# stecrotti/MatrixProductBP.jl

Hardware: AMD Instinct MI355X
Metric: edge-message updates/sec (and s/sweep), SIS 3-regular N=1024 T=50 d=20 (higher is better)
Workload: dtype f64

## Files before the change

### matrixproductbp.jl_amd/csrc/engine.h

```cpp
#if !defined(WG_THREADS)
#error "engine.h is included from kernels.h, once per workgroup-size variant"
#endif

namespace eng {

using namespace wg;

__device__ __forceinline__ int r16(int x) { return (x + 15) & ~15; }
__device__ __forceinline__ int r32(int x) { return (x + 31) & ~31; }

typedef __attribute__((address_space(1))) int32_t gint;
typedef __attribute__((address_space(3))) int lint;

template <class DP>
__device__ inline void stage_core(DP dst, const gdbl* base, const gint* bond, int64_t stride, int L,
                                  int t, bool mirror, int nyq) {
  const int tp = mirror ? (L - 1 - t) : t;
  const int pl = bond[tp], pr = bond[tp + 1];
  const int a = mirror ? pr : pl, an = mirror ? pl : pr;
  const gdbl* src = base + (int64_t)tp * stride;
  const int tot = a * an * nyq;
  for (int idx = threadIdx.x; idx < tot; idx += WG_THREADS) {
    int m = idx % a; int rest = idx / a; int n = rest % an; int s = rest / an;
    int mp = mirror ? n : m, np_ = mirror ? m : n;
    dst[idx] = src[mp + pl * (np_ + pr * s)];
  }
}

template <class DP>
__device__ inline void build_E(DP E, DP A2c, const gdbl* pyy, int b, int bn, int ny, int ny1,
                               int ny2, int q) {
  const int M2 = b * ny, K2 = bn * ny1;
  const int tot = M2 * K2 * q;
  for (int idx = threadIdx.x; idx < tot; idx += WG_THREADS) {
    int i = idx % M2; int rest = idx / M2; int kk = rest % K2; int xi = rest / K2;
    int m2 = i % b, y = i / b, n2 = kk % bn, y1 = kk / bn;
    double s = 0.0;
    for (int y2 = 0; y2 < ny2; y2++) {
      double c = pyy[y + ny * (y1 + ny1 * (y2 + ny2 * xi))];
      if (c != 0.0) s += c * A2c[m2 + b * (n2 + bn * (y2 + ny2 * xi))];
    }
    E[idx] = s;
  }
}

__device__ inline void atomic_max_double_pos(unsigned long long* addr, double v) {
  atomicMax(addr, (unsigned long long)__double_as_longlong(v));
}

template <bool CORES_LDS, bool JAC_LDS, bool EXT>
__device__ void run_problem(const EngProb& P, const EngCfg& cfg, double* slot_, double* lds_, EngStats* stats) {
  typedef typename std::conditional<CORES_LDS, ldbl*, gdbl*>::type CP;
  typedef typename std::conditional<JAC_LDS, ldbl*, gdbl*>::type JP;
  const int tid = threadIdx.x;
  const int L = cfg.L;
  const bool mirror = P.mirror != 0;
  const int ny1 = P.ny1, ny2 = P.ny2, ny = P.ny, q = P.q;
  gdbl* slot = (gdbl*)slot_;
  ldbl* lds = (ldbl*)lds_;
  ldbl* ldsG = lds + cfg.lds_gemm;
  ldbl* ldsQ = lds + cfg.lds_qr;
  ldbl* misc = lds + cfg.lds_misc;
  CP A1c = CORES_LDS ? (CP)(lds + cfg.lds_A1c) : (CP)(slot + cfg.off_A1c);
  CP A2c = CORES_LDS ? (CP)(lds + cfg.lds_A2c) : (CP)(slot + cfg.off_A2c);
  CP E = CORES_LDS ? (CP)(lds + cfg.lds_E) : (CP)(slot + cfg.off_E);
  JP JA = JAC_LDS ? (JP)(lds + cfg.lds_JA) : (JP)(slot + cfg.off_JA);
  lint* rdim = (lint*)(lds + cfg.lds_rdim);
  ldbl* red = misc;
  ldbl* sig = misc + 32;
  lint* ord = (lint*)(misc + 32 + cfg.nmax);
  gdbl* LfS = slot + cfg.off_Lf;
  gdbl* Z = slot + cfg.off_Z;
  gdbl* Y = slot + cfg.off_Y;
  gdbl* T1 = slot + cfg.off_T1;
  gdbl* Nt = slot + cfg.off_Nt;
  gdbl* Mt = slot + cfg.off_Mt;
  gdbl* Ccur = slot + cfg.off_C0;
  gdbl* Cnew = slot + cfg.off_C1;
  const gdbl* PA1 = (const gdbl*)P.A1; const gdbl* PA2 = (const gdbl*)P.A2;
  const gint* Pb1 = (const gint*)P.bond1; const gint* Pb2 = (const gint*)P.bond2;
  const gdbl* Ppyy = (const gdbl*)P.pyy;
  gdbl* Pout = (gdbl*)P.out; gint* Pob = (gint*)P.obond;

  auto LB1 = [&](int t) { return mirror ? Pb1[L - t] : Pb1[t]; };
  auto LB2 = [&](int t) { return mirror ? Pb2[L - t] : Pb2[t]; };
  auto TP = [&](int t) { return mirror ? (L - 1 - t) : t; };
  constexpr bool ext = EXT;
  const gdbl* Plf = (const gdbl*)P.lf;
  const __attribute__((address_space(1))) int64_t* Plfoff = (const __attribute__((address_space(1))) int64_t*)P.lfoff;
  const gint* Prd = (const gint*)P.rdim;
  auto RD = [&](int t) -> int { return ext ? (int)Prd[t] : (int)rdim[t]; };
  auto LFP = [&](int t) -> const gdbl* { return ext ? Plf + Plfoff[t] : (const gdbl*)(LfS + (int64_t)t * cfg.lf_stride); };
  Prof* pr = cfg.prof;
  unsigned long long plast = pr ? wall_clock64() : 0ULL;
#define PROF(ph) prof_mark(pr, plast, ph)

  if (tid == 0 && !ext) { rdim[L] = 1; LfS[(int64_t)L * cfg.lf_stride] = 1.0; }
  __syncthreads();
  for (int t = ext ? 0 : L - 1; t >= 1; t--) {
    const int a = LB1(t), an = LB1(t + 1), b = LB2(t), bn = LB2(t + 1);
    const int Bm = a * b, Bn = an * bn;
    const int r1 = rdim[t + 1];
    const gdbl* Lf1 = LfS + (int64_t)(t + 1) * cfg.lf_stride;
    stage_core(A1c, PA1, Pb1, P.stride1, L, t, mirror, ny1 * q);
    stage_core(A2c, PA2, Pb2, P.stride2, L, t, mirror, ny2 * q);
    __syncthreads();
    build_E(E, A2c, Ppyy + (int64_t)TP(t) * P.pyy_tstride, b, bn, ny, ny1, ny2, q);
    __syncthreads();
    PROF(PH_STAGE);
    const int M1 = a * ny1 * q;
    const int64_t zld = (int64_t)r1 * bn;
    gemm_direct<false, true>(M1, r1 * bn, an, A1c,
         [=](int i) { return (i % a) + a * an * (i / a); }, [=](int kk) { return a * kk; },
         Lf1, [=](int kk) { return (int64_t)r1 * kk; },
         [=](int j) { return (int64_t)(j % r1) + (int64_t)r1 * an * (j / r1); },
         Z, [=](int i) { return zld * i; }, [=](int j) { return (int64_t)j; }, false);
    PROF(PH_Y1);
    const int rowsY = r1 * ny * q;
    const int ldY = r32(rowsY);
    const int cols16 = r16(Bm) + 16;
    for (int64_t idx = tid; idx < (int64_t)(ldY - rowsY) * cols16; idx += WG_THREADS) {
      int rr = rowsY + (int)(idx % (ldY - rowsY)); int64_t c = idx / (ldY - rowsY);
      Y[rr + (int64_t)ldY * c] = 0.0;
    }
    for (int64_t idx = tid; idx < (int64_t)ldY * (cols16 - Bm); idx += WG_THREADS)
      Y[(int64_t)ldY * Bm + idx] = 0.0;
    const int M2 = b * ny, K2 = bn * ny1;
    for (int xi = 0; xi < q; xi++) {
      gemm_direct<true, true>(M2, r1 * a, K2, E + (int64_t)xi * M2 * K2,
           [=](int i) { return i; }, [=](int kk) { return M2 * kk; },
           Z + zld * a * ny1 * xi,
           [=](int kk) { return (int64_t)r1 * (kk % bn) + zld * a * (kk / bn); },
           [=](int j) { return (int64_t)(j % r1) + zld * (j / r1); },
           Y + (int64_t)r1 * ny * xi,
           [=](int i) { return (int64_t)r1 * (i / b) + (int64_t)ldY * a * (i % b); },
           [=](int j) { return (int64_t)(j % r1) + (int64_t)ldY * (j / r1); }, false);
    }
    PROF(PH_Y2);
    qr_r(Y, ldY, rowsY, Bm, ldsQ, ldsG, pr, &plast, PH_QR1_PANEL, PH_QR1_TRAIL, cfg.force_generic != 0);
    const int kmax = min(rowsY, Bm);
    const int lane_ = tid & 63, wave_ = __builtin_amdgcn_readfirstlane(tid >> 6);
    constexpr int LFC = 4;
    double mx = 0.0;
    for (int m0 = LFC * wave_; m0 < Bm; m0 += LFC * WG_WAVES) {
      const int kcap = min(kmax, m0 + LFC);
      for (int k = lane_; k < kcap; k += 64) {
        double v[LFC];
#pragma unroll
        for (int c = 0; c < LFC; c++) {
          const int m = min(m0 + c, Bm - 1);
          v[c] = Y[(int64_t)ldY * m + min(k, min(kmax, m + 1) - 1)];
        }
#pragma unroll
        for (int c = 0; c < LFC; c++) mx = fmax(mx, fabs(v[c]));
      }
    }
    mx = wg_max(mx, red);
    const double inv = (mx > 0.0 && isfinite(mx)) ? 1.0 / mx : 1.0;
    gdbl* Lf0 = LfS + (int64_t)t * cfg.lf_stride;
    for (int m0 = LFC * wave_; m0 < Bm; m0 += LFC * WG_WAVES) {
      for (int k = lane_; k < kmax; k += 64) {
        double v[LFC];
#pragma unroll
        for (int c = 0; c < LFC; c++) {
          const int m = min(m0 + c, Bm - 1);
          v[c] = Y[(int64_t)ldY * m + min(k, min(kmax, m + 1) - 1)];
        }
#pragma unroll
        for (int c = 0; c < LFC; c++) {
          const int m = m0 + c;
          if (m < Bm) Lf0[(int64_t)kmax * m + k] = (k < min(kmax, m + 1)) ? v[c] * inv : 0.0;
        }
      }
    }
    if (tid == 0) rdim[t] = kmax;
    __syncthreads();
    PROF(PH_LF);
  }

  double logc = 0.0;
  int kc = 1;
  if (tid == 0) Ccur[0] = 1.0;
  if (tid == 0) { Pob[mirror ? L : 0] = 1; Pob[mirror ? 0 : L] = 1; }
  __syncthreads();
  for (int t = 0; t < L; t++) {
    const int a = LB1(t), an = LB1(t + 1), b = LB2(t), bn = LB2(t + 1);
    const int Bn = an * bn;
    const int tp = TP(t);
    stage_core(A1c, PA1, Pb1, P.stride1, L, t, mirror, ny1 * q);
// ... 3 lines not shown
    __syncthreads();
    PROF(PH_STAGE);
    const int MT1 = an * ny1 * q;
    const int64_t tld = (int64_t)kc * b;
    gemm_direct(MT1, kc * b, a, A1c,
         [=](int i) { return a * (i % an) + a * an * (i / an); }, [=](int kk) { return kk; },
         Ccur, [=](int kk) { return (int64_t)kc * kk; },
         [=](int j) { return (int64_t)(j % kc) + (int64_t)kc * a * (j / kc); },
         T1, [=](int i) { return tld * i; }, [=](int j) { return (int64_t)j; }, false);
    const int Rr = kc * ny * q;
    const int M2 = b * ny, K2 = bn * ny1;
    for (int xi = 0; xi < q; xi++) {
      gemm_direct(bn * ny, kc * an, b * ny1, E + (int64_t)xi * M2 * K2,
           [=](int i) { return b * (i / bn) + M2 * (i % bn); },
           [=](int kk) { return (kk % b) + M2 * bn * (kk / b); },
           T1 + tld * an * ny1 * xi,
           [=](int kk) { return (int64_t)kc * (kk % b) + tld * an * (kk / b); },
           [=](int j) { return (int64_t)(j % kc) + tld * (j / kc); },
           Nt + (int64_t)kc * ny * xi,
           [=](int i) { return (int64_t)kc * (i / bn) + (int64_t)Rr * an * (i % bn); },
           [=](int j) { return (int64_t)(j % kc) + (int64_t)Rr * (j / kc); }, false);
    }
    {
      double mx = wg_maxabs(Nt, Rr, Rr, Bn, red);
      if (!(mx == mx) || isinf(mx)) { if (tid == 0) stats->nan_flag = 1; }
      if (mx > 0.0 && isfinite(mx)) {
        const double inv = 1.0 / mx;
        for (int64_t idx = tid; idx < (int64_t)Rr * Bn; idx += WG_THREADS) Nt[idx] *= inv;
        logc += log(mx);
      }
      __syncthreads();
    }
    PROF(PH_N);
    gdbl* oc = Pout + (int64_t)tp * P.ostride;
    if (t == L - 1) {
      for (int idx = tid; idx < Rr; idx += WG_THREADS) {
        int k = idx % kc, s = idx / kc;
        oc[k + kc * s] = Nt[idx];
      }
      __syncthreads();
      break;
    }
    const int r1 = RD(t + 1);
    const gdbl* Lf1 = LFP(t + 1);
    const int ldM = r32(r1);
    const int Rr16 = r16(Rr) + 16;
    for (int64_t idx = tid; idx < (int64_t)(ldM - r1) * Rr16; idx += WG_THREADS) {
      int rr = r1 + (int)(idx % (ldM - r1)); int64_t c = idx / (ldM - r1);
      Mt[rr + (int64_t)ldM * c] = 0.0;
    }
    for (int64_t idx = tid; idx < (int64_t)ldM * (Rr16 - Rr); idx += WG_THREADS) Mt[(int64_t)ldM * Rr + idx] = 0.0;
    gemm(Rr, r1, Bn, Nt, [=](int i) { return (int64_t)i; }, [=](int kk) { return (int64_t)Rr * kk; },
         Lf1, [=](int kk) { return (int64_t)r1 * kk; }, [=](int j) { return j; }, false,
         Mt, [=](int i) { return (int64_t)ldM * i; }, [=](int j) { return j; }, false, ldsG);
    PROF(PH_MT);
    qr_r(Mt, ldM, r1, Rr, ldsQ, ldsG, pr, &plast, PH_QR2_PANEL, PH_QR2_TRAIL, cfg.force_generic != 0);
    const int k2 = min(r1, Rr);
    const int ldJ = JAC_LDS ? (Rr | 1) : ((Rr + 15) & ~15);
    double fro2 = 0.0;
    for (int idx = tid; idx < k2 * Rr; idx += WG_THREADS) {
      int r = idx % Rr, c = idx / Rr;
      double v = (r >= c) ? Mt[c + (int64_t)ldM * r] : 0.0;
      JA[r + ldJ * c] = v;
      fro2 += v * v;
    }
    fro2 = wg_sum(fro2, red);
    __syncthreads();
    const int sw = jacobi_rsv(JA, ldJ, Rr, k2, nullptr, 0, red, ord, 60);
    if (tid == 0) {
      if (sw < 0) stats->jacobi_fail = 1;
      atomicAdd(&stats->jac_sweeps, (unsigned long long)(sw < 0 ? 60 : sw));
      atomicAdd(&stats->jac_calls, 1ULL);
    }
    PROF(PH_JAC);
    const double nul2 = 1e-28 * fro2;
    for (int c = tid; c < Rr; c += WG_THREADS) sig[c] = 0.0;
    __syncthreads();
    for (int c = tid; c < k2; c += WG_THREADS) {
      double s = 0.0;
      for (int r = 0; r < Rr; r++) { double v = JA[r + ldJ * c]; s += v * v; }
      const bool ok = s > nul2 && s > 0.0;
      const double sg = ok ? sqrt(s) : 0.0, inv = ok ? 1.0 / sqrt(s) : 0.0;
      for (int r = 0; r < Rr; r++) JA[r + ldJ * c] *= inv;
      sig[c] = sg;
    }
    __syncthreads();
    for (int c = tid; c < k2; c += WG_THREADS) {
      const double sc = sig[c];
      int rank = 0;
      for (int j = 0; j < k2; j++) { double sj = sig[j]; rank += (sj > sc) || (sj == sc && j < c); }
      ord[rank] = c;
    }
    __syncthreads();
    const int len = min(Rr, r1);
    int kp;
    {
      double tot = 0.0;
      for (int j = 0; j < len; j++) { double s = sig[ord[j]]; tot += s * s; }
      const mpbp_trunc tr = cfg.trunc;
      int kth = len;
      if (tr.kind == MPBP_TRUNC_THRESH || tr.kind == MPBP_TRUNC_BOND_THRESH) {
        const double thr = tr.eps * sqrt(tot);
        kth = 0;
        for (int j = 0; j < len; j++) if (sig[ord[j]] > thr) kth = j + 1;
        if (kth < 1) kth = 1;
      }
      if (tr.kind == MPBP_TRUNC_THRESH) kp = kth;
// ... 54 lines not shown
```

### matrixproductbp.jl_amd/csrc/mpbp_hip.hip

```cpp
#include <chrono>
#include "kernels.h"
#include "ctx.h"
#include "v2_engine.h"

thread_local std::string g_create_error;

extern "C" const char* mpbp_last_error(const mpbp_ctx* ctx) { return ctx ? ctx->err.c_str() : g_create_error.c_str(); }

extern "C" int mpbp_create(mpbp_ctx** out, const mpbp_desc* d) {
  if (!out || !d) { g_create_error = "null argument"; return MPBP_EINVAL; }
  *out = nullptr;
  if (d->n_nodes <= 0 || d->n_edges <= 0 || d->T < 1 || d->q < 1 || d->q > 4 || d->max_bond < 1 || !d->nbr_ptr ||
      !d->in_edge || !d->out_edge) { g_create_error = "invalid descriptor (need n_nodes,n_edges>0, T>=1, 1<=q<=4, max_bond>=1)"; return MPBP_EINVAL; }
  mpbp_ctx* c = new mpbp_ctx();
  c->N = d->n_nodes; c->E = d->n_edges; c->T = d->T; c->L = d->T + 1; c->q = d->q; c->cap = d->max_bond; c->device = d->device; c->periodic = d->periodic != 0;
  c->nbr_ptr.assign(d->nbr_ptr, d->nbr_ptr + c->N + 1);
  const int nnz = c->nbr_ptr[c->N];
  c->in_edge.assign(d->in_edge, d->in_edge + nnz);
  c->out_edge.assign(d->out_edge, d->out_edge + nnz);
  for (int p = 0; p < nnz; p++)
    if (c->in_edge[p] < 0 || c->in_edge[p] >= c->E || c->out_edge[p] < 0 || c->out_edge[p] >= c->E) {
      g_create_error = "edge id out of range"; delete c; return MPBP_EINVAL;
    }
  c->nslots = d->n_slots > 0 ? d->n_slots : c->E;
// ... 352 lines not shown
      std::vector<double> w((size_t)L * q * q * q * nyc);
      for (int t = 0; t < L; t++)
        for (int y1 = 0; y1 < nyc; y1++)
          for (int xj = 0; xj < q; xj++)
            for (int x = 0; x < q; x++)
              for (int xn = 0; xn < q; xn++) {
                double val;
                if (xj >= QD(eo)) val = 0.0;
                else if (t == L - 1 && !c->periodic) val = PHI(i, t, x);
                else {
                  double s = 0.0;
                  for (int y = 0; y < nyz; y++)
                    for (int y2 = 0; y2 < ny1; y2++) {
                      const double pyy = PYY(t, z - 1, 1, y, y1, y2, x);
                      if (pyy != 0.0) s += PY(t, xn, x, y) * PXY(t, k, y2, xj, x) * pyy;
                    }
                  val = s * PHI(i, t, x);
                }
                w[(size_t)t * q * q * q * nyc + xn + q * (x + q * (xj + (size_t)q * y1))] = val;
              }
      c->wmsg_off[p] = ts.add(w);
    }
    {
      std::vector<double> w((size_t)L * q * q * nyz);
      for (int t = 0; t < L; t++)
        for (int y = 0; y < nyz; y++)
          for (int x = 0; x < q; x++)
            for (int xn = 0; xn < q; xn++)
              w[(size_t)t * q * q * nyz + xn + q * (x + (size_t)q * y)] = (t == L - 1 && !c->periodic) ? PHI(i, t, x) : PY(t, xn, x, y) * PHI(i, t, x);
      c->wbel_off[i] = ts.add(w);
    }
  }
  if (c->d_tab) { hipFree(c->d_tab); c->d_tab = nullptr; }
  c->tab_doubles = ts.data.size();
  HIPCHK(c, hipMalloc(&c->d_tab, sizeof(double) * std::max<size_t>(ts.data.size(), 4)));
  HIPCHK(c, hipMemcpy(c->d_tab, ts.data.data(), sizeof(double) * ts.data.size(), hipMemcpyHostToDevice));
  c->tables_dirty = false;
  return MPBP_OK;
}

#define RCCHK(call) do { const int rc_ = (call); if (rc_ != MPBP_OK) return rc_; } while (0)

namespace {

enum Form { FORM_AUTO, FORM_GRID, FORM_WG };

struct SweepEnv {
  int split_nodes = 0;
  bool force_generic = false;
  bool no_small = false;
  bool force_small = false;
  bool no_pack = false;
  bool coop_fail_once = false;
  Form gauge = FORM_AUTO, sweep2 = FORM_AUTO;
};
static SweepEnv read_sweep_env() {
  auto set = [](const char* name) { return getenv(name) != nullptr; };
  auto is1 = [](const char* name) { const char* e = getenv(name); return e && e[0] == '1'; };
  auto form = [](const char* name) { const char* e = getenv(name); return !e ? FORM_AUTO : !strcmp(e, "grid") ? FORM_GRID : !strcmp(e, "wg") ? FORM_WG : FORM_AUTO; };
  const char* split = getenv("MPBP_DEBUG_SPLIT_NODES");
  return SweepEnv{split ? atoi(split) : 0, is1("MPBP_DEBUG_FORCE_GENERIC"), is1("MPBP_DEBUG_NO_SMALL"), set("MPBP_DEBUG_FORCE_SMALL"),
                  set("MPBP_DEBUG_NO_PACK"), set("MPBP_DEBUG_COOP_FAIL_ONCE"), form("MPBP_GAUGE"), form("MPBP_SWEEP2")};
}
struct Pass {
  mpbp_ctx* c; const SweepEnv& env; mpbp_trunc trunc; double damp;
  float ms_orth = 0.f; int n_orth = 0;
};
struct OpRec { int in1, in2, out, d1, d2, node, level; };

struct TrainSpec { int cap, ny, qphys; int d; int level; int64_t tab_off; bool is_init; int node; int kron_skip = -2; };
struct NodePlan { int node; std::vector<int> src, dest; int full; int init; };
struct FinRec { int k, j, p, src, ct, out; int nrm = -1, sum = -1, out2 = -1, occ = 0; bool gen = false; };
struct SweepPlan {
  std::vector<TrainSpec> specs;
  std::vector<OpRec> ops;
  std::vector<NodePlan> plans;
  std::vector<FinRec> fins, bels;
  int maxlevel = 0;
  bool any_generic = false;
};
struct EventPair {
  hipEvent_t a = nullptr, b = nullptr;
  EventPair() { hipEventCreate(&a); hipEventCreate(&b); }
  ~EventPair() { if (a) hipEventDestroy(a); if (b) hipEventDestroy(b); }
  EventPair(const EventPair&) = delete;
  EventPair& operator=(const EventPair&) = delete;
};

struct EngLaunchPlan {
  std::vector<EngProb> probs; std::vector<double> cost;
  int cap1 = 1, cap2 = 1, ny1 = 1, ny2 = 1, ny = 1, q = 1, capout = 1;
  bool small = false;
  bool ext = false;
};

static inline bool small_problem(const SweepEnv& env, int64_t B, int ny, int q) {
  return !env.no_small && B * ny * q <= v64::wg::QR_RS * 64;
}

static inline int r16h(int x) { return (x + 15) & ~15; }
static size_t free_bytes() { size_t freeb = 0, totb = 0; hipMemGetInfo(&freeb, &totb); return freeb; }

static void plan_cfg(const EngLaunchPlan& pl, int L, mpbp_trunc trunc, bool force_generic, EngCfg& cfg, size_t& lds_bytes) {
  memset(&cfg, 0, sizeof cfg);
  cfg.L = L; cfg.trunc = trunc;
  const int64_t Bmax = (int64_t)pl.cap1 * pl.cap2;
  const int nmax = pl.capout * pl.ny * pl.q;
  cfg.Bmax = (int)Bmax; cfg.nmax = nmax;
  int64_t off = 0;
  auto take = [&](int64_t n) { int64_t o = off; off += (n + 15) & ~int64_t(15); return o; };
  if (pl.ext) { cfg.lf_stride = 16; cfg.off_Lf = take(16); cfg.off_Z = take(16); cfg.off_Y = take(16); }
  else {
    cfg.lf_stride = (Bmax * Bmax + 15) & ~int64_t(15);
    cfg.off_Lf = take(cfg.lf_stride * (L + 1));
    cfg.off_Z = take((int64_t)pl.cap1 * pl.ny1 * pl.q * pl.cap2 * Bmax);
// ... 18 lines not shown
  const int64_t budget = pl.small ? (38 * 1024) / 8 : (158 * 1024) / 8;
  const int64_t base = l;
  const int64_t coresE = ((nA1 + 3) & ~3) + ((nA2 + 3) & ~3) + ((nE + 3) & ~3);
  const int64_t jac = (((int64_t)(nmax + 1) * std::min<int64_t>(nmax, Bmax) + 3) & ~3);
  cfg.force_generic = force_generic ? 1 : 0;
  bool cores_fit = !force_generic && base + coresE <= budget, jac_fit = !force_generic && base + jac <= budget;
  if (cores_fit) { int64_t o = base; cfg.lds_A1c = (int32_t)o; o += (nA1 + 3) & ~3; cfg.lds_A2c = (int32_t)o; o += (nA2 + 3) & ~3; cfg.lds_E = (int32_t)o; }
  else { cfg.lds_A1c = cfg.lds_A2c = cfg.lds_E = -1; }
  if (jac_fit) { cfg.lds_JA = (int32_t)base; cfg.lds_JV = -1; }
  else { cfg.lds_JA = cfg.lds_JV = -1; }
  const int64_t gemm_d = pl.small ? 512 : std::max<int64_t>(v512::wg::GM_LDS_DOUBLES, v512::wg::QR_BIG_DOUBLES);
  cfg.lds_gemm = (int32_t)base;
  int64_t top = base + std::max(gemm_d, std::max(cores_fit ? coresE : 0, jac_fit ? jac : 0));
  lds_bytes = (size_t)top * 8;
}

}

static void choose_variant(const Pass& ps, EngLaunchPlan& pl, int64_t bmact) {
  const mpbp_ctx* c = ps.c;
  const int nprob = (int)pl.probs.size();
  if (!pl.small && !ps.env.no_small && (int64_t)pl.cap1 * pl.cap2 * pl.ny * pl.q <= v64::wg::QR_RS * 64 && nprob > 2 * c->num_cu) pl.small = true;
  if (pl.small && nprob <= 2 * c->num_cu && !ps.env.force_small) pl.small = false;
  bool grid = false;
  if (!pl.small) {
    const int64_t Bm = (int64_t)pl.cap1 * pl.cap2;
    if (ps.env.gauge != FORM_AUTO) grid = ps.env.gauge == FORM_GRID;
    else grid = bmact * pl.ny * pl.q > 2048 || Bm * Bm * (c->L + 1) * 8 > (int64_t)256 << 20;
    for (const EngProb& P : pl.probs) if (P.mirror) grid = false;
  }
  pl.ext = grid;
}
static int launch_slots(Pass& ps, const EngLaunchPlan& pl, const EngProb* probs, int np, bool cavity, hipEvent_t e0) {
  mpbp_ctx* c = ps.c;
  EngCfg cfg; size_t lds_bytes;
  plan_cfg(pl, c->L, ps.trunc, ps.env.force_generic, cfg, lds_bytes);
  static const bool prof_small = [] { const char* e = getenv("MPBP_PROF_SMALL"); return e && e[0] == '1'; }();
  cfg.prof = (c->profiling >= 2 && (prof_small ? pl.small : cavity)) ? c->d_prof : nullptr;
  auto kern = pl.small ? v64::eng_kernel : v512::eng_kernel;
  const int nthreads = pl.small ? 64 : 512;
  HIPCHK(c, hipFuncSetAttribute((const void*)kern, hipFuncAttributeMaxDynamicSharedMemorySize, (int)lds_bytes));
  int per_cu = 1;
  hipOccupancyMaxActiveBlocksPerMultiprocessor(&per_cu, kern, nthreads, lds_bytes);
  if (per_cu < 1) per_cu = 1;
  int nslots = std::min(np, c->num_cu * per_cu);
  size_t slot_bytes = (size_t)cfg.slot_doubles * 8;
  size_t budget = c->scratch.cap + (size_t)(free_bytes() * 0.85);
  while (nslots > 1 && (size_t)nslots * slot_bytes > budget) nslots = (nslots + 1) / 2;
  RCCHK(ensure_arena(c, c->scratch, (size_t)nslots * slot_bytes + sizeof(EngProb) * np + 4096));
  double* d_scr = (double*)c->scratch.base;
  EngProb* d_probs = (EngProb*)(c->scratch.base + (((size_t)nslots * slot_bytes + 255) & ~size_t(255)));
  HIPCHK(c, hipMemcpyAsync(d_probs, probs, sizeof(EngProb) * np, hipMemcpyHostToDevice, c->stream));
  HIPCHK(c, hipMemsetAsync(c->d_counter, 0, sizeof(int), c->stream));
  if (e0) hipEventRecord(e0, c->stream);
  hipLaunchKernelGGL(kern, dim3(nslots), dim3(nthreads), lds_bytes, c->stream, d_probs, np, c->d_counter, cfg, d_scr, c->d_stats);
  HIPCHK(c, hipGetLastError());
  return MPBP_OK;
}
static int launch_grid(Pass& ps, const EngLaunchPlan& pl, std::vector<EngProb>& probs, const std::vector<int32_t>& hb, int64_t bmact, bool cavity) {
  mpbp_ctx* c = ps.c;
  const int nprob = (int)probs.size();
  const bool plannable = ps.trunc.kind == MPBP_TRUNC_BOND || ps.trunc.kind == MPBP_TRUNC_BOND_MAX;
  bool s2grid = plannable && 2.0 * (double)bmact * (double)bmact * pl.capout * pl.ny * pl.q >= 2e8;
  if (ps.env.sweep2 != FORM_AUTO) s2grid = plannable && ps.env.sweep2 == FORM_GRID;
  for (int done = 0; done < nprob;) {
    int nd = 0, did2 = 0;
    for (int attempt = 0;; attempt++) {
      EngStats sbak;
      const bool may_retry = !c->no_coop_panel;
      if (may_retry) HIPCHK(c, hipMemcpyAsync(&sbak, c->d_stats, sizeof sbak, hipMemcpyDeviceToHost, c->stream));
      RCCHK(v2_gauge_sweep(c, probs.data() + done, nprob - done, hb.data() + (size_t)done * 2 * (c->L + 1), s2grid ? &ps.trunc : nullptr, &nd, &did2));
      if (!did2) RCCHK(launch_slots(ps, pl, probs.data() + done, nd, cavity, nullptr));
      HIPCHK(c, hipStreamSynchronize(c->stream));
      int herr = 0;
      HIPCHK(c, hipMemcpy(&herr, c->d_counter + 8, sizeof(int), hipMemcpyDeviceToHost));
      if (ps.env.coop_fail_once && may_retry && attempt == 0) herr = 1;
      if (!herr) break;
      if (!may_retry) return c->fail(MPBP_EHIP, "batched gauge sweep: arrival counter timed out although the cooperative panel kernel was not used");
      c->no_coop_panel = true;
      HIPCHK(c, hipMemcpy(c->d_stats, &sbak, sizeof sbak, hipMemcpyHostToDevice));
    }
    done += nd;
  }
  return MPBP_OK;
}
static int launch_engine_impl(Pass& ps, EngLaunchPlan& pl, bool cavity) {
  mpbp_ctx* c = ps.c;
  const int nprob = (int)pl.probs.size();
  if (nprob == 0) return MPBP_OK;
  std::vector<int> idx(nprob);
  for (int i = 0; i < nprob; i++) idx[i] = i;
  std::stable_sort(idx.begin(), idx.end(), [&](int a, int b) { return pl.cost[a] > pl.cost[b]; });
  std::vector<EngProb> sorted(nprob);
  for (int i = 0; i < nprob; i++) sorted[i] = pl.probs[idx[i]];
  std::vector<int32_t> hb;
  RCCHK(v2_gather_bonds(c, sorted.data(), nprob, hb));
  const int L1 = c->L + 1;
  int a1 = 1, a2 = 1; int64_t bmact = 1;
  for (int i = 0; i < nprob; i++) {
    const int32_t* b1 = hb.data() + (size_t)i * 2 * L1; const int32_t* b2 = b1 + L1;
    for (int t = 0; t < L1; t++) { a1 = std::max(a1, (int)b1[t]); a2 = std::max(a2, (int)b2[t]); bmact = std::max<int64_t>(bmact, (int64_t)b1[t] * b2[t]); }
  }
  pl.cap1 = std::min(pl.cap1, a1); pl.cap2 = std::min(pl.cap2, a2);
  choose_variant(ps, pl, bmact);
  const bool timed = cavity && c->profiling;
  EventPair lev;
// ... 730 lines not shown
```

### matrixproductbp.jl_amd/csrc/wg_blocks.h

```cpp
#if !defined(WG_THREADS) || !defined(WG_WAVES)
#error "define WG_THREADS / WG_WAVES and include wg_common.h before wg_blocks.h (see kernels.h)"
#endif

namespace wg {

using namespace wgc;

constexpr int GM_MB = 96;
constexpr int GM_NT = 128;
constexpr int GM_KC = 32;
constexpr int GM_LDA = 112;
constexpr int GM_LDB = 144;
constexpr int GM_LDS_DOUBLES = GM_KC * (GM_LDA + GM_LDB);

template <bool NTX = false, bool NTO = false, class SP, class XP, class OP, class SRO, class SCO, class XRO, class XCO,
          class ORO, class OCO>
__device__ __attribute__((noinline)) void gemm_direct(int M, int N, int K, SP Sp, SRO sro, SCO sco,
                                                     XP Xp, XRO xro, XCO xco, OP Op, ORO oro, OCO oco,
                                                     bool accumulate, int tile0 = -1, int tstride = WG_WAVES);

template <class SRO, class SCO, class XRO, class XCO, class ORO, class OCO>
__device__ __attribute__((noinline)) void gemm(int M, int N, int K, const gdbl* Sp, SRO sro, SCO sco, const gdbl* Xp, XRO xro,
                     XCO xco, bool xkfast, gdbl* Op, ORO oro, OCO oco, bool accumulate, ldbl* lds) {
#if WG_THREADS != 512
  (void)xkfast; (void)lds;
  gemm_direct<false, false>(M, N, K, Sp, sro, sco, Xp, xro, xco, Op, oro, oco, accumulate);
#else
  const int tid = threadIdx.x;
  const int lane = tid & 63, wave = __builtin_amdgcn_readfirstlane(tid >> 6);
  const int g = lane >> 4, l15 = lane & 15;
  ldbl* As = lds;
  ldbl* Bs = lds + GM_KC * GM_LDA;
  for (int mb = 0; mb < M; mb += GM_MB) {
    const int mrows = min(GM_MB, M - mb);
    const int ntm = (mrows + 15) >> 4;
    const int si = tid & 127;
    const bool s_act = si < ntm * 16;
    const bool s_in = si < mrows;
    const long s_ro = s_in ? (long)sro(mb + si) : 0;
    for (int n0 = 0; n0 < N; n0 += GM_NT) {
      const int ncols = min(GM_NT, N - n0);
      constexpr int NE = GM_KC / 4;
      constexpr int JS = 512 / GM_KC;
      long x_co[NE];
      bool x_in[NE];
      if (xkfast) {
#pragma unroll
        for (int e = 0; e < NE; e++) {
          int j = tid / GM_KC + JS * e;
          x_in[e] = j < ncols;
          x_co[e] = x_in[e] ? (long)xco(n0 + j) : 0;
        }
      } else {
        int j = tid & 127;
        x_in[0] = j < ncols;
        x_co[0] = x_in[0] ? (long)xco(n0 + j) : 0;
      }
      d4 acc[6];
#pragma unroll
      for (int t = 0; t < 6; t++) acc[t] = d4{0, 0, 0, 0};
      const bool w_act = wave * 16 < ncols;
      double sv[NE], xv[NE];
      auto load_chunk = [&](int k0) {
#pragma unroll
        for (int e = 0; e < NE; e++) {
          const int kk = (tid >> 7) + 4 * e;
          const bool ok = s_in && k0 + kk < K;
          const double v = Sp[s_ro + (long)sco(ok ? k0 + kk : 0)];
          sv[e] = ok ? v : 0.0;
        }
        if (xkfast) {
          const int kk = tid % GM_KC;
          const bool kin = k0 + kk < K;
          const long r = (long)xro(kin ? k0 + kk : 0);
#pragma unroll
          for (int e = 0; e < NE; e++) {
            const double v = Xp[r + x_co[e]];
            xv[e] = (kin && x_in[e]) ? v : 0.0;
          }
        } else {
#pragma unroll
          for (int e = 0; e < NE; e++) {
            const int kk = (tid >> 7) + 4 * e;
            const bool ok = x_in[0] && k0 + kk < K;
            const double v = Xp[(long)xro(ok ? k0 + kk : 0) + x_co[0]];
            xv[e] = ok ? v : 0.0;
          }
        }
      };
      load_chunk(0);
      for (int k0 = 0; k0 < K; k0 += GM_KC) {
        if (s_act) {
#pragma unroll
          for (int e = 0; e < NE; e++) As[((tid >> 7) + 4 * e) * GM_LDA + si] = sv[e];
        }
        if (xkfast) {
#pragma unroll
          for (int e = 0; e < NE; e++) Bs[(tid % GM_KC) * GM_LDB + tid / GM_KC + JS * e] = xv[e];
        } else {
#pragma unroll
          for (int e = 0; e < NE; e++) Bs[((tid >> 7) + 4 * e) * GM_LDB + (tid & 127)] = xv[e];
        }
        __syncthreads();
        if (k0 + GM_KC < K) load_chunk(k0 + GM_KC);
        if (w_act) {
#pragma unroll
          for (int ks = 0; ks < GM_KC / 4; ks++) {
            const int krow = ks * 4 + g;
            const double b = Bs[krow * GM_LDB + wave * 16 + l15];
#pragma unroll
            for (int t = 0; t < 6; t++) {
              if (t < ntm) {
                const double a = As[krow * GM_LDA + t * 16 + l15];
                acc[t] = mfma(a, b, acc[t]);
              }
            }
          }
        }
        __syncthreads();
      }
      if (w_act) {
        const int col = wave * 16 + l15;
        if (col < ncols) {
          const long oc = (long)oco(n0 + col);
#pragma unroll
          for (int t = 0; t < 6; t++) {
            if (t < ntm) {
#pragma unroll
              for (int r = 0; r < 4; r++) {
                int row = t * 16 + g + 4 * r;
                if (row < mrows) {
                  gdbl* p = Op + (long)oro(mb + row) + oc;
                  double v = acc[t][r];
                  if (accumulate) v += *p;
                  *p = v;
                }
              }
            }
          }
        }
      }
    }
  }
  __syncthreads();
#endif
}

template <bool NTX, bool NTO, class SP, class XP, class OP, class SRO, class SCO, class XRO, class XCO, class ORO, class OCO>
__device__ __attribute__((noinline)) void gemm_direct(int M, int N, int K, SP Sp, SRO sro, SCO sco,
                                                     XP Xp, XRO xro, XCO xco, OP Op, ORO oro, OCO oco,
                                                     bool accumulate, int tile0, int tstride) {
  const int tid = threadIdx.x;
  const int lane = tid & 63, wave = __builtin_amdgcn_readfirstlane(tid >> 6);
  const int g = lane >> 4, l15 = lane & 15;
  const int nks = (K + 3) >> 2;
  const int ntile = (N + 15) >> 4;
  for (int mb = 0; mb < M; mb += GM_MB) {
    const int mrows = min(GM_MB, M - mb);
    const int ntm = (mrows + 15) >> 4;
    long s_ro[6];
    bool s_in[6];
#pragma unroll
    for (int t = 0; t < 6; t++) {
      const int i = t * 16 + l15;
      s_in[t] = t < ntm && i < mrows;
      s_ro[t] = s_in[t] ? (long)sro(mb + i) : 0;
    }
    struct Grp { double b[5]; long so[5]; unsigned kin; };
    auto fetch = [&](long cofs, int ks0, Grp& G) {
      G.kin = 0;
#pragma unroll
      for (int u = 0; u < 5; u++) {
        const int k = 4 * (ks0 + u) + g;
        const bool kin = (ks0 + u < nks) && k < K;
        const int kc = kin ? k : 0;
        G.b[u] = NTX ? __builtin_nontemporal_load(Xp + ((long)xro(kc) + cofs)) : Xp[(long)xro(kc) + cofs];
        G.so[u] = (long)sco(kc);
        G.kin |= kin ? (1u << u) : 0u;
      }
    };
    auto tiles = [&](auto ntm_c) {
      constexpr int NTM = decltype(ntm_c)::value;
      int tl = tile0 < 0 ? wave : tile0;
      if (tl >= ntile) return;
      int j = tl * 16 + l15;
      bool jin = j < N;
      long cofs = jin ? (long)xco(j) : 0;
      Grp cur, nxt;
      fetch(cofs, 0, cur);
      for (;;) {
        d4 acc[NTM];
#pragma unroll
        for (int t = 0; t < NTM; t++) acc[t] = d4{0, 0, 0, 0};
        const int tl2 = tl + tstride;
        const int j2 = tl2 * 16 + l15;
        const bool jin2 = j2 < N;
        long cofs2 = 0;
        for (int ks0 = 0; ks0 < nks; ks0 += 5) {
          if (ks0 + 5 < nks) fetch(cofs, ks0 + 5, nxt);
          else if (tl2 < ntile) { cofs2 = jin2 ? (long)xco(j2) : 0; fetch(cofs2, 0, nxt); }
#pragma unroll
          for (int u = 0; u < 5; u++) {
            const bool kin = (cur.kin >> u) & 1u;
            const double bv = (kin && jin) ? cur.b[u] : 0.0;
#pragma unroll
            for (int t = 0; t < NTM; t++) acc[t] = mfma(Sp[s_ro[t] + cur.so[u]], bv, acc[t]);
          }
          cur = nxt;
        }
        if (jin) {
          const long oc = (long)oco(j);
#pragma unroll
          for (int t = 0; t < NTM; t++) {
#pragma unroll
            for (int r = 0; r < 4; r++) {
              const int row = t * 16 + g + 4 * r;
              if (row < mrows) {
                OP p = Op + (long)oro(mb + row) + oc;
                double v = acc[t][r];
                if (accumulate) v += *p;
                if (NTO) __builtin_nontemporal_store(v, p); else *p = v;
              }
            }
          }
        }
        tl = tl2;
        if (tl >= ntile) break;
        j = j2; jin = jin2; cofs = cofs2;
      }
    };
    constexpr int NGC = 2;
    if (nks <= 5 * NGC) {
      long xr_[NGC][5], so_[NGC][5];
      unsigned kinm[NGC];
#pragma unroll
      for (int gi = 0; gi < NGC; gi++) {
        kinm[gi] = 0;
#pragma unroll
        for (int u = 0; u < 5; u++) {
          const int k = 4 * (5 * gi + u) + g;
          const bool kin = (5 * gi + u < nks) && k < K;
          const int kc = kin ? k : 0;
          xr_[gi][u] = (long)xro(kc);
          so_[gi][u] = (long)sco(kc);
          kinm[gi] |= kin ? (1u << u) : 0u;
        }
      }
      auto tiles_c = [&](auto ntm_c) {
        constexpr int NTM = decltype(ntm_c)::value;
        int tl = tile0 < 0 ? wave : tile0;
        if (tl >= ntile) return;
        int j = tl * 16 + l15;
        bool jin = j < N;
        long cofs = jin ? (long)xco(j) : 0;
        double cb[5], nb[5];
        auto fetchc = [&](long co, int gi, double (&b)[5]) {
#pragma unroll
          for (int u = 0; u < 5; u++) {
            const long o = (gi == 0 ? xr_[0][u] : xr_[NGC - 1][u]) + co;
            b[u] = NTX ? __builtin_nontemporal_load(Xp + o) : Xp[o];
          }
        };
        fetchc(cofs, 0, cb);
        for (;;) {
          d4 acc[NTM];
#pragma unroll
          for (int t = 0; t < NTM; t++) acc[t] = d4{0, 0, 0, 0};
          const int tl2 = tl + tstride;
          const int j2 = tl2 * 16 + l15;
          const bool jin2 = j2 < N;
          long cofs2 = 0;
#pragma unroll
          for (int gi = 0; gi < NGC; gi++) {
            if (5 * gi >= nks) break;
            if (gi + 1 < NGC && 5 * (gi + 1) < nks) fetchc(cofs, gi + 1, nb);
            else if (tl2 < ntile) { cofs2 = jin2 ? (long)xco(j2) : 0; fetchc(cofs2, 0, nb); }
#pragma unroll
            for (int u = 0; u < 5; u++) {
              const bool kin = (kinm[gi] >> u) & 1u;
              const double bv = (kin && jin) ? cb[u] : 0.0;
#pragma unroll
              for (int t = 0; t < NTM; t++) acc[t] = mfma(Sp[s_ro[t] + so_[gi][u]], bv, acc[t]);
            }
#pragma unroll
            for (int u = 0; u < 5; u++) cb[u] = nb[u];
          }
          if (jin) {
            const long oc = (long)oco(j);
#pragma unroll
            for (int t = 0; t < NTM; t++) {
#pragma unroll
              for (int r = 0; r < 4; r++) {
                const int row = t * 16 + g + 4 * r;
                if (row < mrows) {
                  OP p = Op + (long)oro(mb + row) + oc;
                  double v = acc[t][r];
                  if (accumulate) v += *p;
                  if (NTO) __builtin_nontemporal_store(v, p); else *p = v;
                }
              }
            }
          }
          tl = tl2;
          if (tl >= ntile) break;
          j = j2; jin = jin2; cofs = cofs2;
        }
      };
      switch (ntm) {
        case 1: tiles_c(std::integral_constant<int, 1>{}); break;
        case 2: tiles_c(std::integral_constant<int, 2>{}); break;
        case 3: tiles_c(std::integral_constant<int, 3>{}); break;
        case 4: tiles_c(std::integral_constant<int, 4>{}); break;
        case 5: tiles_c(std::integral_constant<int, 5>{}); break;
        default: tiles_c(std::integral_constant<int, 6>{}); break;
      }
      continue;
    }
    switch (ntm) {
      case 1: tiles(std::integral_constant<int, 1>{}); break;
      case 2: tiles(std::integral_constant<int, 2>{}); break;
      case 3: tiles(std::integral_constant<int, 3>{}); break;
      case 4: tiles(std::integral_constant<int, 4>{}); break;
      case 5: tiles(std::integral_constant<int, 5>{}); break;
      default: tiles(std::integral_constant<int, 6>{}); break;
    }
  }
  __syncthreads();
}

__device__ __forceinline__ double wave_sum(double v) {
#pragma unroll
  for (int o = 32; o > 0; o >>= 1) v += __shfl_xor(v, o, 64);
  return v;
}
__device__ __forceinline__ double wave_max(double v) {
#pragma unroll
  for (int o = 32; o > 0; o >>= 1) v = fmax(v, __shfl_xor(v, o, 64));
  return v;
}

__device__ __forceinline__ double wg_sum(double v, ldbl* red) {
  v = wave_sum(v);
  __syncthreads();
  if ((threadIdx.x & 63) == 0) red[threadIdx.x >> 6] = v;
  __syncthreads();
  double s = 0;
#pragma unroll
  for (int w = 0; w < WG_WAVES; w++) s += red[w];
  return s;
}
__device__ __forceinline__ double wg_max(double v, ldbl* red) {
  v = wave_max(v);
  __syncthreads();
  if ((threadIdx.x & 63) == 0) red[threadIdx.x >> 6] = v;
  __syncthreads();
  double s = red[0];
#pragma unroll
  for (int w = 1; w < WG_WAVES; w++) s = fmax(s, red[w]);
// ... 1622 lines not shown
```

Baseline: 574.3.

## Exploit triangular zero structure of Lf in GEMMs to skip tiles and loads

Adds zero-pattern predicates describing where the Lf factor (an upper-triangular R factor from QR) is structurally zero. The GEMM kernels use them to skip whole output tiles (Y1), skip leading K chunks (LDS GEMM for Mt), and suppress global loads for zero K-steps (Y2, Mt) via wave ballots. The aim is to cut wasted MFMA work and memory traffic on known zeros. The cost is extra per-tile and per-load predicate and ballot work, plus a correctness dependence on the triangular assumption, for which a debug poison-Z option is added.

```diff
diff --git a/matrixproductbp.jl_amd/csrc/engine.h b/matrixproductbp.jl_amd/csrc/engine.h
--- a/matrixproductbp.jl_amd/csrc/engine.h
+++ b/matrixproductbp.jl_amd/csrc/engine.h
@@ -43,6 +43,32 @@
     E[idx] = s;
   }
 }
+
+__device__ __forceinline__ bool lf_zero(int k, int m) { return m < k; }
+__device__ __forceinline__ int z_run_end(int an, int n2) { return an * (n2 + 1) - 1; }
+__device__ __forceinline__ bool z_zero(int an, int k, int n2) { return lf_zero(k, z_run_end(an, n2)); }
+struct LfZeroY1 {
+  static constexpr bool on = true, skip_tiles = true, skip_ksteps = false;
+  int an, r1;
+  __device__ __forceinline__ int xm(int n1) const { return n1; }
+  __device__ __forceinline__ int xk(int j) const { return (j % r1) - an * (j / r1); }
+  __device__ __forceinline__ bool z(int xk_, int xm_) const { return lf_zero(xk_, xm_); }
+};
+struct LfZeroY2 {
+  static constexpr bool on = true, skip_tiles = false, skip_ksteps = true;
+  static constexpr int xm_none = -1, xk_none = 0x7fffffff;
+  int an, bn, r1;
+  __device__ __forceinline__ int xm(int kk) const { return z_run_end(an, kk % bn); }
+  __device__ __forceinline__ int xk(int j) const { return j % r1; }
+  __device__ __forceinline__ bool z(int k, int mend) const { return lf_zero(k, mend); }
+};
+struct LfZeroMt {
+  static constexpr bool on = true, skip_tiles = false, skip_ksteps = true;
+  static constexpr int xm_none = -1, xk_none = 0x7fffffff;
+  __device__ __forceinline__ int xm(int m) const { return m; }
+  __device__ __forceinline__ int xk(int k) const { return k; }
+  __device__ __forceinline__ bool z(int k, int m) const { return lf_zero(k, m); }
+};
 
 __device__ inline void atomic_max_double_pos(unsigned long long* addr, double v) {
   atomicMax(addr, (unsigned long long)__double_as_longlong(v));
@@ -114,7 +140,7 @@
          [=](int i) { return (i % a) + a * an * (i / a); }, [=](int kk) { return a * kk; },
          Lf1, [=](int kk) { return (int64_t)r1 * kk; },
          [=](int j) { return (int64_t)(j % r1) + (int64_t)r1 * an * (j / r1); },
-         Z, [=](int i) { return zld * i; }, [=](int j) { return (int64_t)j; }, false);
+         Z, [=](int i) { return zld * i; }, [=](int j) { return (int64_t)j; }, false, -1, WG_WAVES, LfZeroY1{an, r1});
     PROF(PH_Y1);
     const int rowsY = r1 * ny * q;
     const int ldY = r32(rowsY);
@@ -134,7 +160,7 @@
            [=](int j) { return (int64_t)(j % r1) + zld * (j / r1); },
            Y + (int64_t)r1 * ny * xi,
            [=](int i) { return (int64_t)r1 * (i / b) + (int64_t)ldY * a * (i % b); },
-           [=](int j) { return (int64_t)(j % r1) + (int64_t)ldY * (j / r1); }, false);
+           [=](int j) { return (int64_t)(j % r1) + (int64_t)ldY * (j / r1); }, false, -1, WG_WAVES, LfZeroY2{an, bn, r1});
     }
     PROF(PH_Y2);
     qr_r(Y, ldY, rowsY, Bm, ldsQ, ldsG, pr, &plast, PH_QR1_PANEL, PH_QR1_TRAIL, cfg.force_generic != 0);
@@ -244,7 +270,7 @@
     for (int64_t idx = tid; idx < (int64_t)ldM * (Rr16 - Rr); idx += WG_THREADS) Mt[(int64_t)ldM * Rr + idx] = 0.0;
     gemm(Rr, r1, Bn, Nt, [=](int i) { return (int64_t)i; }, [=](int kk) { return (int64_t)Rr * kk; },
          Lf1, [=](int kk) { return (int64_t)r1 * kk; }, [=](int j) { return j; }, false,
-         Mt, [=](int i) { return (int64_t)ldM * i; }, [=](int j) { return j; }, false, ldsG);
+         Mt, [=](int i) { return (int64_t)ldM * i; }, [=](int j) { return j; }, false, ldsG, LfZeroMt{});
     PROF(PH_MT);
     qr_r(Mt, ldM, r1, Rr, ldsQ, ldsG, pr, &plast, PH_QR2_PANEL, PH_QR2_TRAIL, cfg.force_generic != 0);
     const int k2 = min(r1, Rr);
diff --git a/matrixproductbp.jl_amd/csrc/mpbp_hip.hip b/matrixproductbp.jl_amd/csrc/mpbp_hip.hip
--- a/matrixproductbp.jl_amd/csrc/mpbp_hip.hip
+++ b/matrixproductbp.jl_amd/csrc/mpbp_hip.hip
@@ -428,6 +428,7 @@
   bool force_small = false;
   bool no_pack = false;
   bool coop_fail_once = false;
+  bool poison_z = false;
   Form gauge = FORM_AUTO, sweep2 = FORM_AUTO;
 };
 static SweepEnv read_sweep_env() {
@@ -436,7 +437,7 @@
   auto form = [](const char* name) { const char* e = getenv(name); return !e ? FORM_AUTO : !strcmp(e, "grid") ? FORM_GRID : !strcmp(e, "wg") ? FORM_WG : FORM_AUTO; };
   const char* split = getenv("MPBP_DEBUG_SPLIT_NODES");
   return SweepEnv{split ? atoi(split) : 0, is1("MPBP_DEBUG_FORCE_GENERIC"), is1("MPBP_DEBUG_NO_SMALL"), set("MPBP_DEBUG_FORCE_SMALL"),
-                  set("MPBP_DEBUG_NO_PACK"), set("MPBP_DEBUG_COOP_FAIL_ONCE"), form("MPBP_GAUGE"), form("MPBP_SWEEP2")};
+                  set("MPBP_DEBUG_NO_PACK"), set("MPBP_DEBUG_COOP_FAIL_ONCE"), is1("MPBP_DEBUG_POISON_Z"), form("MPBP_GAUGE"), form("MPBP_SWEEP2")};
 }
 struct Pass {
   mpbp_ctx* c; const SweepEnv& env; mpbp_trunc trunc; double damp;
@@ -561,6 +562,8 @@
   EngProb* d_probs = (EngProb*)(c->scratch.base + (((size_t)nslots * slot_bytes + 255) & ~size_t(255)));
   HIPCHK(c, hipMemcpyAsync(d_probs, probs, sizeof(EngProb) * np, hipMemcpyHostToDevice, c->stream));
   HIPCHK(c, hipMemsetAsync(c->d_counter, 0, sizeof(int), c->stream));
+  if (ps.env.poison_z)
+    HIPCHK(c, hipMemset2DAsync(d_scr + cfg.off_Z, slot_bytes, 0xFF, (size_t)(cfg.off_Y - cfg.off_Z) * 8, (size_t)nslots, c->stream));
   if (e0) hipEventRecord(e0, c->stream);
   hipLaunchKernelGGL(kern, dim3(nslots), dim3(nthreads), lds_bytes, c->stream, d_probs, np, c->d_counter, cfg, d_scr, c->d_stats);
   HIPCHK(c, hipGetLastError());
diff --git a/matrixproductbp.jl_amd/csrc/wg_blocks.h b/matrixproductbp.jl_amd/csrc/wg_blocks.h
--- a/matrixproductbp.jl_amd/csrc/wg_blocks.h
+++ b/matrixproductbp.jl_amd/csrc/wg_blocks.h
@@ -13,18 +13,20 @@
 constexpr int GM_LDB = 144;
 constexpr int GM_LDS_DOUBLES = GM_KC * (GM_LDA + GM_LDB);
 
+struct NoZeros { static constexpr bool on = false, skip_tiles = false, skip_ksteps = false; };
+
 template <bool NTX = false, bool NTO = false, class SP, class XP, class OP, class SRO, class SCO, class XRO, class XCO,
-          class ORO, class OCO>
+          class ORO, class OCO, class ZP = NoZeros>
 __device__ __attribute__((noinline)) void gemm_direct(int M, int N, int K, SP Sp, SRO sro, SCO sco,
                                                      XP Xp, XRO xro, XCO xco, OP Op, ORO oro, OCO oco,
-                                                     bool accumulate, int tile0 = -1, int tstride = WG_WAVES);
-
-template <class SRO, class SCO, class XRO, class XCO, class ORO, class OCO>
+                                                     bool accumulate, int tile0 = -1, int tstride = WG_WAVES, ZP zp = ZP{});
+
+template <class SRO, class SCO, class XRO, class XCO, class ORO, class OCO, class ZP = NoZeros>
 __device__ __attribute__((noinline)) void gemm(int M, int N, int K, const gdbl* Sp, SRO sro, SCO sco, const gdbl* Xp, XRO xro,
-                     XCO xco, bool xkfast, gdbl* Op, ORO oro, OCO oco, bool accumulate, ldbl* lds) {
+                     XCO xco, bool xkfast, gdbl* Op, ORO oro, OCO oco, bool accumulate, ldbl* lds, ZP zp = ZP{}) {
 #if WG_THREADS != 512
   (void)xkfast; (void)lds;
-  gemm_direct<false, false>(M, N, K, Sp, sro, sco, Xp, xro, xco, Op, oro, oco, accumulate);
+  gemm_direct<false, false>(M, N, K, Sp, sro, sco, Xp, xro, xco, Op, oro, oco, accumulate, -1, WG_WAVES, zp);
 #else
   const int tid = threadIdx.x;
   const int lane = tid & 63, wave = __builtin_amdgcn_readfirstlane(tid >> 6);
@@ -88,8 +90,13 @@
           }
         }
       };
-      load_chunk(0);
-      for (int k0 = 0; k0 < K; k0 += GM_KC) {
+      int kbeg = 0;
+      if constexpr (ZP::on) {
+        const int xk0 = zp.xk(n0);
+        while (kbeg < K && zp.z(xk0, zp.xm(min(kbeg + GM_KC, K) - 1))) kbeg += GM_KC;
+      }
+      load_chunk(kbeg);
+      for (int k0 = kbeg; k0 < K; k0 += GM_KC) {
         if (s_act) {
 #pragma unroll
           for (int e = 0; e < NE; e++) As[((tid >> 7) + 4 * e) * GM_LDA + si] = sv[e];
@@ -146,15 +153,27 @@
 #endif
 }
 
-template <bool NTX, bool NTO, class SP, class XP, class OP, class SRO, class SCO, class XRO, class XCO, class ORO, class OCO>
+template <bool NTX, bool NTO, class SP, class XP, class OP, class SRO, class SCO, class XRO, class XCO, class ORO, class OCO, class ZP>
 __device__ __attribute__((noinline)) void gemm_direct(int M, int N, int K, SP Sp, SRO sro, SCO sco,
                                                      XP Xp, XRO xro, XCO xco, OP Op, ORO oro, OCO oco,
-                                                     bool accumulate, int tile0, int tstride) {
+                                                     bool accumulate, int tile0, int tstride, ZP zp) {
   const int tid = threadIdx.x;
   const int lane = tid & 63, wave = __builtin_amdgcn_readfirstlane(tid >> 6);
   const int g = lane >> 4, l15 = lane & 15;
   const int nks = (K + 3) >> 2;
   const int ntile = (N + 15) >> 4;
+  constexpr bool ZT = ZP::on && ZP::skip_tiles, ZK = ZP::on && ZP::skip_ksteps;
+  auto live_tile = [&](int tl) {
+    if constexpr (ZT) {
+      const int xm_last = zp.xm(K - 1);
+      while (tl < ntile) {
+        const int j = tl * 16 + l15;
+        if (__ballot(j < N && !zp.z(zp.xk(j < N ? j : 0), xm_last)) != 0) break;
+        tl += tstride;
+      }
+    }
+    return tl;
+  };
   for (int mb = 0; mb < M; mb += GM_MB) {
     const int mrows = min(GM_MB, M - mb);
     const int ntm = (mrows + 15) >> 4;
@@ -167,42 +186,57 @@
       s_ro[t] = s_in[t] ? (long)sro(mb + i) : 0;
     }
     struct Grp { double b[5]; long so[5]; unsigned kin; };
-    auto fetch = [&](long cofs, int ks0, Grp& G) {
+    auto fetch = [&](long cofs, int ks0, Grp& G, int xk, bool jn) {
       G.kin = 0;
 #pragma unroll
       for (int u = 0; u < 5; u++) {
         const int k = 4 * (ks0 + u) + g;
         const bool kin = (ks0 + u < nks) && k < K;
         const int kc = kin ? k : 0;
-        G.b[u] = NTX ? __builtin_nontemporal_load(Xp + ((long)xro(kc) + cofs)) : Xp[(long)xro(kc) + cofs];
-        G.so[u] = (long)sco(kc);
-        G.kin |= kin ? (1u << u) : 0u;
+        if constexpr (ZK) {
+          const bool use = kin && jn && !zp.z(xk, zp.xm(kc));
+          G.kin |= use ? (1u << u) : 0u;
+          long o = (long)xro(kc) + cofs;
+          if (__ballot(use) == 0) o = 0;
+          G.b[u] = NTX ? __builtin_nontemporal_load(Xp + o) : Xp[o];
+          G.so[u] = (long)sco(kc);
+        } else {
+          G.b[u] = NTX ? __builtin_nontemporal_load(Xp + ((long)xro(kc) + cofs)) : Xp[(long)xro(kc) + cofs];
+          G.so[u] = (long)sco(kc);
+          G.kin |= kin ? (1u << u) : 0u;
+        }
       }
     };
     auto tiles = [&](auto ntm_c) {
       constexpr int NTM = decltype(ntm_c)::value;
-      int tl = tile0 < 0 ? wave : tile0;
+      int tl = live_tile(tile0 < 0 ? wave : tile0);
       if (tl >= ntile) return;
       int j = tl * 16 + l15;
       bool jin = j < N;
       long cofs = jin ? (long)xco(j) : 0;
+      int xk = 0, xk2 = 0;
+      if constexpr (ZK) xk = zp.xk(jin ? j : 0);
       Grp cur, nxt;
-      fetch(cofs, 0, cur);
+      fetch(cofs, 0, cur, xk, jin);
       for (;;) {
         d4 acc[NTM];
 #pragma unroll
         for (int t = 0; t < NTM; t++) acc[t] = d4{0, 0, 0, 0};
-        const int tl2 = tl + tstride;
+        const int tl2 = live_tile(tl + tstride);
         const int j2 = tl2 * 16 + l15;
         const bool jin2 = j2 < N;
         long cofs2 = 0;
         for (int ks0 = 0; ks0 < nks; ks0 += 5) {
-          if (ks0 + 5 < nks) fetch(cofs, ks0 + 5, nxt);
-          else if (tl2 < ntile) { cofs2 = jin2 ? (long)xco(j2) : 0; fetch(cofs2, 0, nxt); }
+          if (ks0 + 5 < nks) fetch(cofs, ks0 + 5, nxt, xk, jin);
+          else if (tl2 < ntile) {
+            cofs2 = jin2 ? (long)xco(j2) : 0;
+            if constexpr (ZK) xk2 = zp.xk(jin2 ? j2 : 0);
+            fetch(cofs2, 0, nxt, xk2, jin2);
+          }
 #pragma unroll
           for (int u = 0; u < 5; u++) {
             const bool kin = (cur.kin >> u) & 1u;
-            const double bv = (kin && jin) ? cur.b[u] : 0.0;
+            const double bv = (kin && (ZK || jin)) ? cur.b[u] : 0.0;
 #pragma unroll
             for (int t = 0; t < NTM; t++) acc[t] = mfma(Sp[s_ro[t] + cur.so[u]], bv, acc[t]);
           }
@@ -226,13 +260,14 @@
         }
         tl = tl2;
         if (tl >= ntile) break;
-        j = j2; jin = jin2; cofs = cofs2;
+        j = j2; jin = jin2; cofs = cofs2; xk = xk2;
       }
     };
     constexpr int NGC = 2;
     if (nks <= 5 * NGC) {
       long xr_[NGC][5], so_[NGC][5];
       unsigned kinm[NGC];
+      int xm_[NGC][5];
 #pragma unroll
       for (int gi = 0; gi < NGC; gi++) {
         kinm[gi] = 0;
@@ -244,41 +279,53 @@
           xr_[gi][u] = (long)xro(kc);
           so_[gi][u] = (long)sco(kc);
           kinm[gi] |= kin ? (1u << u) : 0u;
+          if constexpr (ZK) xm_[gi][u] = kin ? zp.xm(kc) : ZP::xm_none;
         }
       }
       auto tiles_c = [&](auto ntm_c) {
         constexpr int NTM = decltype(ntm_c)::value;
-        int tl = tile0 < 0 ? wave : tile0;
+        int tl = live_tile(tile0 < 0 ? wave : tile0);
         if (tl >= ntile) return;
         int j = tl * 16 + l15;
         bool jin = j < N;
         long cofs = jin ? (long)xco(j) : 0;
         double cb[5], nb[5];
-        auto fetchc = [&](long co, int gi, double (&b)[5]) {
+        int xk = 0, xk2 = 0;
+        if constexpr (ZK) xk = jin ? zp.xk(j) : ZP::xk_none;
+        auto fetchc = [&](long co, int gi, double (&b)[5], int xkt) {
 #pragma unroll
           for (int u = 0; u < 5; u++) {
-            const long o = (gi == 0 ? xr_[0][u] : xr_[NGC - 1][u]) + co;
+            long o = (gi == 0 ? xr_[0][u] : xr_[NGC - 1][u]) + co;
+            if constexpr (ZK) { if (__ballot(!zp.z(xkt, gi == 0 ? xm_[0][u] : xm_[NGC - 1][u])) == 0) o = 0; }
             b[u] = NTX ? __builtin_nontemporal_load(Xp + o) : Xp[o];
           }
         };
-        fetchc(cofs, 0, cb);
+        fetchc(cofs, 0, cb, xk);
         for (;;) {
           d4 acc[NTM];
 #pragma unroll
           for (int t = 0; t < NTM; t++) acc[t] = d4{0, 0, 0, 0};
-          const int tl2 = tl + tstride;
+          const int tl2 = live_tile(tl + tstride);
           const int j2 = tl2 * 16 + l15;
           const bool jin2 = j2 < N;
           long cofs2 = 0;
 #pragma unroll
           for (int gi = 0; gi < NGC; gi++) {
             if (5 * gi >= nks) break;
-            if (gi + 1 < NGC && 5 * (gi + 1) < nks) fetchc(cofs, gi + 1, nb);
-            else if (tl2 < ntile) { cofs2 = jin2 ? (long)xco(j2) : 0; fetchc(cofs2, 0, nb); }
+            if (gi + 1 < NGC && 5 * (gi + 1) < nks) fetchc(cofs, gi + 1, nb, xk);
+            else if (tl2 < ntile) {
+              cofs2 = jin2 ? (long)xco(j2) : 0;
+              if constexpr (ZK) xk2 = jin2 ? zp.xk(j2) : ZP::xk_none;
+              fetchc(cofs2, 0, nb, xk2);
+            }
 #pragma unroll
             for (int u = 0; u < 5; u++) {
-              const bool kin = (kinm[gi] >> u) & 1u;
-              const double bv = (kin && jin) ? cb[u] : 0.0;
+              double bv;
+              if constexpr (ZK) bv = zp.z(xk, xm_[gi][u]) ? 0.0 : cb[u];
+              else {
+                const bool kin = (kinm[gi] >> u) & 1u;
+                bv = (kin && jin) ? cb[u] : 0.0;
+              }
 #pragma unroll
               for (int t = 0; t < NTM; t++) acc[t] = mfma(Sp[s_ro[t] + so_[gi][u]], bv, acc[t]);
             }
@@ -303,7 +350,7 @@
           }
           tl = tl2;
           if (tl >= ntile) break;
-          j = j2; jin = jin2; cofs = cofs2;
+          j = j2; jin = jin2; cofs = cofs2; xk = xk2;
         }
       };
       switch (ntm) {
```

After: 596.9, median of 6. 3.9% higher.
